# lukedan/libfluid

Measured on AMD Instinct MI355X. Metric: particle_steps_per_sec, higher is better.
Workload: dtype f32

## Files before the change

libfluid_amd/csrc/core.hip:

```cpp
#include <math.h>

#include <algorithm>
#include <stdarg.h>
#include <stdio.h>
#include <string.h>

#include <mutex>

#include "common.h"
#include "pcg.h"
#include "stream_set.h"

static thread_local std::string g_create_error;

int lfa_fail(lfa_sim *s, int code, const char *fmt, ...) {
	char buf[512];
	va_list ap;
	va_start(ap, fmt);
	vsnprintf(buf, sizeof buf, fmt, ap);
	va_end(ap);
	if (s) s->err = buf;
	else g_create_error = buf;
	return code;
}
// ... 744 lines not shown
	return LFA_OK;
}

__global__ void k_set_solid(const int32_t *xyz, size_t k, uint8_t *solid, uint8_t *ctype, GridDims g) {
	size_t i = (size_t)blockIdx.x * blockDim.x + threadIdx.x;
	if (i >= k) return;
	int x = xyz[3 * i], y = xyz[3 * i + 1], z = xyz[3 * i + 2];
	if (!in_grid(g, x, y, z)) return;
	uint32_t b = blocked_index(g, x, y, z);
	solid[b] = 1;
	ctype[b] = CT_SOLID;
}

extern "C" int lfa_set_solid_cells(lfa_sim *s, const int32_t *xyz, uint64_t k) {
	if (!s || (!xyz && k)) return LFA_E_INVALID;
	++s->solid_epoch;
	if (k == 0) return LFA_OK;
	LFA_HIP(s, hipSetDevice(s->device));
	LFA_TRY(lfa_corr_commit(s));
	LFA_TRY(lfa_ensure_io(s, k * 12));
	LFA_HIP(s, hipMemcpyAsync(s->io_buf, xyz, k * 12, hipMemcpyHostToDevice, s->stream));
	hipLaunchKernelGGL(k_set_solid, dim3((unsigned)((k + 255) / 256)), dim3(256), 0, s->stream,
	                   (const int32_t *)s->io_buf, (size_t)k, s->solid, s->ctype, s->g);
	LFA_LAUNCH_CHECK(s);
	LFA_HIP(s, hipStreamSynchronize(s->stream));
	s->system_valid = false;
	return LFA_OK;
}

extern "C" int lfa_clear_solid_cells(lfa_sim *s) {
	if (!s) return LFA_E_INVALID;
	++s->solid_epoch;
	LFA_HIP(s, hipSetDevice(s->device));
	LFA_TRY(lfa_corr_commit(s));
	hipLaunchKernelGGL(k_init_ctype, dim3((unsigned)((s->ncp + 255) / 256)), dim3(256), 0, s->stream, s->ctype, s->solid,
	                   s->g, s->ncp);
	LFA_LAUNCH_CHECK(s);
	s->system_valid = false;
	s->grid_valid = false;
	return LFA_OK;
}

struct CellAos {
	double vel[3];
	uint8_t type;
	uint8_t pad[7];
};

__global__ void k_export_cells(CellAos *out, GridDims g, size_t nc, CellView cv) {
	size_t r = (size_t)blockIdx.x * blockDim.x + threadIdx.x;
	if (r >= nc) return;
	int x = (int)(r % g.nx), y = (int)((r / g.nx) % g.ny), z = (int)(r / ((size_t)g.nx * g.ny));
	uint32_t b = blocked_index(g, x, y, z);
	CellAos c;
	memset(&c, 0, sizeof c);
	const int rule = cell_tile_rule(cv, b >> 9);
#pragma unroll
	for (int k = 0; k < 3; ++k) c.vel[k] = cell_velocity(cv, rule, b, k);
	c.type = cell_type(cv, rule, b);
	out[r] = c;
}

static int export_cells(lfa_sim *s, void *aos32, const float *u, const float *v, const float *w, bool old) {
	LFA_HIP(s, hipSetDevice(s->device));
	LFA_TRY(lfa_ensure_io(s, s->nc * 32));
	hipLaunchKernelGGL(k_export_cells, dim3((unsigned)((s->nc + 255) / 256)), dim3(256), 0, s->stream,
	                   (CellAos *)s->io_buf, s->g, s->nc, lfa_cell_view(s, u, v, w, old));
	LFA_LAUNCH_CHECK(s);
	LFA_HIP(s, hipMemcpyAsync(aos32, s->io_buf, s->nc * 32, hipMemcpyDeviceToHost, s->stream));
	LFA_HIP(s, hipStreamSynchronize(s->stream));
	return LFA_OK;
}

extern "C" int lfa_download_cells(lfa_sim *s, void *aos32) {
	if (!s || !aos32) return LFA_E_INVALID;
	return export_cells(s, aos32, s->u, s->v, s->w, false);
}
extern "C" int lfa_download_old_cells(lfa_sim *s, void *aos32) {
	if (!s || !aos32) return LFA_E_INVALID;
	if (!s->uo) return lfa_fail(s, LFA_E_INVALID, "no old grid: FLIP P2G has not run");
	return export_cells(s, aos32, s->uo, s->vo, s->wo, true);
}

__global__ void k_import_cells(const CellAos *in, GridDims g, size_t nc, float *u, float *v, float *w, uint8_t *ctype,
                               uint8_t *solid) {
	size_t r = (size_t)blockIdx.x * blockDim.x + threadIdx.x;
	if (r >= nc) return;
	int x = (int)(r % g.nx), y = (int)((r / g.nx) % g.ny), z = (int)(r / ((size_t)g.nx * g.ny));
	uint32_t b = blocked_index(g, x, y, z);
	CellAos c = in[r];
	u[b] = (float)c.vel[0]; v[b] = (float)c.vel[1]; w[b] = (float)c.vel[2];
	ctype[b] = c.type & 7;
	solid[b] = (c.type & CT_SOLID) ? 1 : 0;
}

extern "C" int lfa_upload_cells(lfa_sim *s, const void *aos32) {
	if (!s || !aos32) return LFA_E_INVALID;
	++s->solid_epoch;
	LFA_HIP(s, hipSetDevice(s->device));
	LFA_TRY(lfa_corr_join(s));
	LFA_TRY(lfa_ensure_io(s, s->nc * 32));
	LFA_HIP(s, hipMemcpyAsync(s->io_buf, aos32, s->nc * 32, hipMemcpyHostToDevice, s->stream));
	hipLaunchKernelGGL(k_import_cells, dim3((unsigned)((s->nc + 255) / 256)), dim3(256), 0, s->stream,
	                   (const CellAos *)s->io_buf, s->g, s->nc, s->u, s->v, s->w, s->ctype, s->solid);
	LFA_LAUNCH_CHECK(s);
	LFA_HIP(s, hipStreamSynchronize(s->stream));
	s->grid_valid = false;
	s->bg[0] = s->bg[1] = s->bg[2] = 0.0;
	s->system_valid = false;
	return LFA_OK;
}

__global__ void __launch_bounds__(256) k_tile_count(const uint32_t *key, size_t n, uint32_t *tile_count, uint32_t *rank) {
	const int lane = threadIdx.x & 63;
	const size_t wave = ((size_t)blockIdx.x * blockDim.x + threadIdx.x) >> 6;
	const size_t i0 = wave * (64 * TC_CHUNKS) + lane;
	uint32_t tile[TC_CHUNKS], my_rank[TC_CHUNKS];
#pragma unroll
	for (int c = 0; c < TC_CHUNKS; ++c) {
		const size_t i = i0 + 64 * c;
		const uint32_t k = i < n ? key[i] : 0xFFFFFFFFu;
		tile[c] = k != 0xFFFFFFFFu ? k >> 9 : 0xFFFFFFFFu;
	}
	lfa_wave_tile_ranks(tile, tile_count, my_rank);
#pragma unroll
	for (int c = 0; c < TC_CHUNKS; ++c) {
		const size_t i = i0 + 64 * c;
		if (tile[c] != 0xFFFFFFFFu) rank[i] = my_rank[c];
	}
}

__global__ void k_tile_flags(const uint32_t *tile_count, uint32_t *flag, int nt) {
	int t = blockIdx.x * blockDim.x + threadIdx.x;
	if (t < nt) flag[t] = tile_count[t] > 0 ? 1u : 0u;
}
__global__ void k_compact_tiles(const uint32_t *flag, const uint32_t *scan, int *list, int *slot_of, int nt) {
	int t = blockIdx.x * blockDim.x + threadIdx.x;
	if (t >= nt) return;
	if (flag[t]) {
		list[scan[t]] = t;
		if (slot_of) slot_of[t] = (int)scan[t];
	} else if (slot_of) {
		slot_of[t] = -1;
	}
}
__global__ void k_dilate(const int *ptiles, int n_ptiles, uint32_t *flag, GridDims g) {
	int i = blockIdx.x * blockDim.x + threadIdx.x;
	if (i >= n_ptiles * 27) return;
	int t = ptiles[i / 27], o = i % 27, tx, ty, tz;
	tile_coords(g, t, tx, ty, tz);
	int x = tx + o % 3 - 1, y = ty + (o / 3) % 3 - 1, z = tz + o / 9 - 1;
	if ((unsigned)x < (unsigned)g.ntx && (unsigned)y < (unsigned)g.nty && (unsigned)z < (unsigned)g.ntz)
		flag[x + g.ntx * (y + g.nty * z)] = 1u;
}

__global__ void k_tile_scatter(size_t n, ParticleSoA src, ParticleSoA dst, const uint32_t *rank,
                               const uint32_t *tile_start, const uint32_t *tile_count, int shuffle, uint32_t *from) {
	size_t i = (size_t)blockIdx.x * blockDim.x + threadIdx.x;
	if (i >= n) return;
	uint32_t key = src.key[i], tile = key >> 9, r = rank[i];
	if (key == 0xFFFFFFFFu) return;
	if (shuffle) {
		uint32_t cnt = tile_count[tile];
		if (cnt % 1000003u != 0) r = (uint32_t)(((uint64_t)r * 1000003ull) % cnt);
	}
	size_t d = (size_t)tile_start[tile] + r;
	dst.key[d] = key;
#pragma unroll
	for (int k = 0; k < 3; ++k) dst.t[k][d] = src.t[k][i];
	dst.id[d] = src.id[i];
	from[d] = (uint32_t)i;
}
__global__ void k_c_to_home(size_t n, ParticleSoA p, float *home, size_t stride) {
	size_t i = (size_t)blockIdx.x * blockDim.x + threadIdx.x;
	if (i >= n || p.key[i] == 0xFFFFFFFFu) return;
	const size_t j = p.id[i];
#pragma unroll
	for (int k = 0; k < 9; ++k) home[k * stride + j] = p.c[k][i];
}
__global__ void k_c_from_home(size_t n, ParticleSoA p, const float *home, size_t stride) {
	size_t i = (size_t)blockIdx.x * blockDim.x + threadIdx.x;
	if (i >= n || p.key[i] == 0xFFFFFFFFu) return;
	const size_t j = p.id[i];
#pragma unroll
	for (int k = 0; k < 9; ++k) p.c[k][i] = home[k * stride + j];
}
__global__ void k_gather_vc(size_t n, ParticleSoA old, ParticleSoA cur, const uint32_t *from, int with_c) {
	size_t d = (size_t)blockIdx.x * blockDim.x + threadIdx.x;
	if (d >= n) return;
	const uint32_t i = from[d];
#pragma unroll
	for (int k = 0; k < 3; ++k) cur.v[k][d] = old.v[k][i];
	if (with_c) {
#pragma unroll
		for (int k = 0; k < 9; ++k) cur.c[k][d] = old.c[k][i];
	}
}

__global__ void __launch_bounds__(256)
k_cell_count(const int *dtiles, int n_dtiles, const uint32_t *key, const uint32_t *tile_start, uint32_t *cell_count) {
	__shared__ uint32_t cnt[LFA_TILE_CELLS];
	for (int slot = blockIdx.x; slot < n_dtiles; slot += gridDim.x) {
		int tile = dtiles[slot];
		cnt[threadIdx.x] = 0;
		cnt[threadIdx.x + 256] = 0;
		__syncthreads();
		uint32_t b = tile_start[tile], e = tile_start[tile + 1];
		for (uint32_t i = b + threadIdx.x; i < e; i += 256) atomicAdd(&cnt[key[i] & 511], 1u);
		__syncthreads();
		cell_count[(size_t)tile * LFA_TILE_CELLS + threadIdx.x] = cnt[threadIdx.x];
		cell_count[(size_t)tile * LFA_TILE_CELLS + 256 + threadIdx.x] = cnt[threadIdx.x + 256];
		__syncthreads();
	}
}

__global__ void k_compact_range(const uint32_t *flag, const uint32_t *scan, int *list, int *slot_of, int lo, int hi,
                                int slot_base) {
	int t = lo + blockIdx.x * blockDim.x + threadIdx.x;
	if (t >= hi) return;
	if (flag[t]) {
		list[scan[t]] = t;
		if (slot_of) slot_of[t] = slot_base + (int)scan[t];
	} else if (slot_of) {
		slot_of[t] = -1;
	}
}
__global__ void k_fill_i32(int *p, int n, int v) {
	int i = blockIdx.x * blockDim.x + threadIdx.x;
	if (i < n) p[i] = v;
}
__global__ void k_gather_u32(const uint32_t *src, const int *idx, int n, uint32_t *dst) {
	int i = threadIdx.x;
	if (i < n) dst[i] = src[idx[i]];
}

__global__ void k_dilate_slots(const int *tile_pslot, uint32_t *flag, GridDims g) {
	const int t = blockIdx.x * blockDim.x + threadIdx.x;
	if (t >= g.nt || tile_pslot[t] < 0) return;
	int tx, ty, tz;
	tile_coords(g, t, tx, ty, tz);
	for (int o = 0; o < 27; ++o) {
		const int x = tx + o % 3 - 1, y = ty + (o / 3) % 3 - 1, z = tz + o / 9 - 1;
		if ((unsigned)x < (unsigned)g.ntx && (unsigned)y < (unsigned)g.nty && (unsigned)z < (unsigned)g.ntz)
			flag[x + g.ntx * (y + g.nty * z)] = 1u;
	}
}

static int compact_tiles_async(lfa_sim *s, const uint32_t *flag, int lo, int hi, int *list, int *slot_of, uint32_t *total_dev) {
	LFA_TRY(lfa_exclusive_scan_u32(s, flag + lo, s->tile_scan + lo, (size_t)(hi - lo), total_dev));
	hipLaunchKernelGGL(k_compact_range, dim3((hi - lo + 255) / 256), dim3(256), 0, s->stream, flag, s->tile_scan - 0,
	                   list - 0, slot_of, lo, hi, 0);
	LFA_LAUNCH_CHECK(s);
	return LFA_OK;
}

int lfa_c_home_ensure(lfa_sim *s, size_t n) {
	if (n <= s->c_home_cap) return LFA_OK;
	const size_t cap = ((n + n / 8) + 1023) & ~(size_t)1023;
	float *nh = nullptr;
	LFA_HIP(s, hipMalloc(&nh, cap * 9 * sizeof(float)));
	auto fail = [&](hipError_t e, const char *what) {
		(void)hipFree(nh);
		return lfa_fail(s, LFA_E_HIP, "%s failed: %s", what, hipGetErrorString(e));
	};
	if (s->c_home && s->c_home_valid && s->c_home_cap)
		for (int k = 0; k < 9; ++k) {
			const hipError_t e = hipMemcpyAsync(nh + (size_t)k * cap, s->c_home + (size_t)k * s->c_home_cap,
			                                    s->c_home_cap * 4, hipMemcpyDeviceToDevice, s->stream);
			if (e != hipSuccess) return fail(e, "copying C to its larger home array");
		}
	if (s->c_home) {
		const hipError_t e = hipStreamSynchronize(s->stream);
		if (e != hipSuccess) return fail(e, "hipStreamSynchronize");
		LFA_HIP(s, hipFree(s->c_home));
	}
	s->c_home = nh;
	s->c_home_cap = cap;
	return LFA_OK;
}
int lfa_c_home_restore(lfa_sim *s) {
	if (!s->c_home_valid) return LFA_OK;
	s->c_home_valid = false;
	const size_t n = s->binned ? s->np_live : s->np;
	if (!n) return LFA_OK;
	hipLaunchKernelGGL(k_c_from_home, dim3((unsigned)((n + 255) / 256)), dim3(256), 0, s->stream, n, s->pb[s->cur], (const float *)s->c_home,
	                   s->c_home_cap);
	LFA_LAUNCH_CHECK(s);
	return LFA_OK;
}

int lfa_particles_materialize(lfa_sim *s) {
	if (!s->vc_pending) return LFA_OK;
	LFA_TRY(lfa_corr_commit(s));
	s->vc_pending = false;
	LFA_HIP(s, hipSetDevice(s->device));
	const size_t n = s->np_live;
	if (!n) return LFA_OK;
	hipLaunchKernelGGL(k_gather_vc, dim3((unsigned)((n + 255) / 256)), dim3(256), 0, s->stream, n, s->pb[s->cur ^ 1], s->pb[s->cur],
	                   (const uint32_t *)s->vc_src, s->vc_with_c ? 1 : 0);
	LFA_LAUNCH_CHECK(s);
	return LFA_OK;
}

extern "C" int lfa_hash_particles(lfa_sim *s) { return lfa_hash_particles_impl(s, false); }
int lfa_hash_particles_impl(lfa_sim *s, bool counts_done) {
	if (!s) return LFA_E_INVALID;
	LFA_HIP(s, hipSetDevice(s->device));
	LFA_TRY(lfa_corr_commit(s));
	LFA_TRY(lfa_particles_materialize(s));
	const GridDims &g = s->g;
	const int nt = g.nt, L = g.ntx * g.nty;
	const size_t n = s->binned ? s->np_live : s->np;
	ParticleSoA &src = s->pb[s->cur], &dst = s->pb[s->cur ^ 1];
	const int own_lo = s->slab_lo * L, own_hi = s->slab_hi * L;
	const int all_lo = lfa_has_lo(s) ? own_lo - L : own_lo, all_hi = lfa_has_hi(s) ? own_hi + L : own_hi;

	if (!counts_done) {
		LFA_HIP(s, hipMemsetAsync(s->tile_count, 0, (size_t)(nt + 1) * 4, s->stream));
		if (n) {
			hipLaunchKernelGGL(k_tile_count, dim3((unsigned)((n + 256 * TC_CHUNKS - 1) / (256 * TC_CHUNKS))), dim3(256), 0, s->stream, src.key, n,
			                   s->tile_count, s->rank);
			LFA_LAUNCH_CHECK(s);
		}
	}
	LFA_TRY(lfa_exclusive_scan_u32(s, s->tile_count, s->tile_start, (size_t)nt + 1, nullptr));
	LFA_HIP(s, hipMemcpyAsync(s->h_pinned + 8, s->tile_start + nt, 4, hipMemcpyDeviceToHost, s->stream));

	hipLaunchKernelGGL(k_tile_flags, dim3((nt + 255) / 256), dim3(256), 0, s->stream, s->tile_count, s->tile_flag, nt);
	LFA_LAUNCH_CHECK(s);
	LFA_TRY(lfa_dist_exchange_tile_layers_u32(s, s->tile_flag));
	hipLaunchKernelGGL(k_fill_i32, dim3((nt + 255) / 256), dim3(256), 0, s->stream, s->tile_pslot, nt, -1);
	LFA_LAUNCH_CHECK(s);
	const bool one_sync = !s->dist;
	if (one_sync) {
		uint32_t *tot = (uint32_t *)s->pcg_state + 8;
		LFA_TRY(compact_tiles_async(s, s->tile_flag, 0, nt, s->ptiles_all, s->tile_pslot, tot));
		LFA_HIP(s, hipMemsetAsync(s->tile_flag, 0, (size_t)(nt + 1) * 4, s->stream));
		hipLaunchKernelGGL(k_dilate_slots, dim3((nt + 255) / 256), dim3(256), 0, s->stream, (const int *)s->tile_pslot, s->tile_flag, g);
		LFA_LAUNCH_CHECK(s);
		LFA_TRY(compact_tiles_async(s, s->tile_flag, 0, nt, s->dtiles, nullptr, tot + 1));
		LFA_HIP(s, hipMemcpyAsync(s->h_pinned + 9, tot, 8, hipMemcpyDeviceToHost, s->stream));
		LFA_HIP(s, hipStreamSynchronize(s->stream));
		s->n_ptiles_all = (int)s->h_pinned[9];
		s->n_dtiles = (int)s->h_pinned[10];
		s->p_off = 0;
		s->n_ptiles = s->n_ptiles_all;
		s->n_own_first = s->n_own_last = s->n_ghost_lo = s->n_ghost_hi = 0;
		s->ptiles = s->ptiles_all;
	} else {
		uint32_t *tot = (uint32_t *)s->pcg_state + 20;
		LFA_TRY(compact_tiles_async(s, s->tile_flag, all_lo, all_hi, s->ptiles_all, s->tile_pslot, tot));
		int marks[4] = {own_lo, own_lo + L < own_hi ? own_lo + L : own_hi, own_hi - L > own_lo ? own_hi - L : own_lo, own_hi};
		int *didx = s->pcg_state + 12;
		LFA_HIP(s, hipMemcpyAsync(didx, marks, 16, hipMemcpyHostToDevice, s->stream));
		hipLaunchKernelGGL(k_gather_u32, dim3(1), dim3(64), 0, s->stream, s->tile_scan, didx, 4, tot + 1);
		LFA_LAUNCH_CHECK(s);
		LFA_HIP(s, hipMemsetAsync(s->tile_flag, 0, (size_t)(nt + 1) * 4, s->stream));
		hipLaunchKernelGGL(k_dilate_slots, dim3((nt + 255) / 256), dim3(256), 0, s->stream, (const int *)s->tile_pslot, s->tile_flag, g);
		LFA_LAUNCH_CHECK(s);
		if (own_lo > 0) LFA_HIP(s, hipMemsetAsync(s->tile_flag, 0, (size_t)own_lo * 4, s->stream));
		if (own_hi < nt) LFA_HIP(s, hipMemsetAsync(s->tile_flag + own_hi, 0, (size_t)(nt - own_hi) * 4, s->stream));
		LFA_TRY(lfa_dist_exchange_tile_layers_u32(s, s->tile_flag));
		LFA_TRY(compact_tiles_async(s, s->tile_flag, own_lo, own_hi, s->dtiles, nullptr, tot + 5));
		{
			const int hlo[4] = {s->slab_lo * L, (s->slab_hi - 1) * L, (s->slab_lo - 1) * L, s->slab_hi * L};
			const bool on[4] = {lfa_has_lo(s), lfa_has_hi(s), lfa_has_lo(s), lfa_has_hi(s)};
			LFA_HIP(s, hipMemsetAsync(tot + 6, 0, 16, s->stream));
			for (int w = 0; w < 4; ++w)
				if (on[w]) LFA_TRY(compact_tiles_async(s, s->tile_flag, hlo[w], hlo[w] + L, s->halo_tiles + (size_t)w * L, nullptr, tot + 6 + w));
		}
		LFA_HIP(s, hipMemcpyAsync(s->h_pinned + 20, tot, 40, hipMemcpyDeviceToHost, s->stream));
		LFA_HIP(s, hipStreamSynchronize(s->stream));
		const uint32_t *h = s->h_pinned + 20;
		s->n_ptiles_all = (int)h[0];
		int vals[4];
		for (int k = 0; k < 4; ++k) vals[k] = marks[k] >= all_hi ? s->n_ptiles_all : (int)h[1 + k];
		s->p_off = vals[0];
		s->n_ptiles = vals[3] - vals[0];
		s->n_own_first = vals[1] - vals[0];
		s->n_own_last = vals[3] - vals[2];
		s->n_ghost_lo = s->p_off;
		s->n_ghost_hi = s->n_ptiles_all - vals[3];
		s->ptiles = s->ptiles_all + s->p_off;
		s->n_dtiles = (int)h[5];
		for (int w = 0; w < 4; ++w) s->n_halo[w] = (int)h[6 + w];
	}
	s->np_live = s->h_pinned[8];
	if (s->dist) s->np = s->np_live;
	s->holes = false;
	s->n_arrivals = 0;
	s->move_pending = false;
	if (n) {
		const dim3 sgrid((unsigned)((n + 255) / 256));
		const bool home = s->prm.simulation_method != LFA_APIC;
		if (home && !s->c_home_valid) {
			LFA_TRY(lfa_c_home_ensure(s, s->dist ? std::max<size_t>(s->pcap, (size_t)s->next_global_id) : s->pcap));
			hipLaunchKernelGGL(k_c_to_home, sgrid, dim3(256), 0, s->stream, n, src, s->c_home, s->c_home_cap);
			LFA_LAUNCH_CHECK(s);
			s->c_home_valid = true;
		} else if (!home && s->c_home_valid) {
			LFA_TRY(lfa_c_home_restore(s));
		}
		hipLaunchKernelGGL(k_tile_scatter, sgrid, dim3(256), 0, s->stream, n, src, dst, s->rank, s->tile_start, s->tile_count,
		                   s->binned ? 0 : 1, s->vc_src);
		LFA_LAUNCH_CHECK(s);
		s->cur ^= 1;
		s->vc_pending = true;
		s->vc_extent = n;
		s->vc_with_c = !home;
	}
	if (s->n_dtiles) {
		int grid = s->n_dtiles < 8192 ? s->n_dtiles : 8192;
		hipLaunchKernelGGL(k_cell_count, dim3(grid), dim3(256), 0, s->stream, s->dtiles, s->n_dtiles,
		                   s->pb[s->cur].key, s->tile_start, s->cell_count);
		LFA_LAUNCH_CHECK(s);
	}
	s->binned = true;
	s->system_valid = false;
	s->unknown_count_valid = false;
	return LFA_OK;
}

int lfa_dist_build_halo_lists(lfa_sim *s, const uint32_t *flag, int *lists, int n[4]) {
	const int L = s->g.ntx * s->g.nty;
	const int lo[4] = {s->slab_lo * L, (s->slab_hi - 1) * L, (s->slab_lo - 1) * L, s->slab_hi * L};
	const bool on[4] = {lfa_has_lo(s), lfa_has_hi(s), lfa_has_lo(s), lfa_has_hi(s)};
	uint32_t *tot = (uint32_t *)s->pcg_state + 26;
	LFA_HIP(s, hipMemsetAsync(tot, 0, 16, s->stream));
	for (int w = 0; w < 4; ++w)
		if (on[w]) LFA_TRY(compact_tiles_async(s, flag, lo[w], lo[w] + L, lists + (size_t)w * L, nullptr, tot + w));
	LFA_HIP(s, hipMemcpyAsync(s->h_pinned + 26, tot, 16, hipMemcpyDeviceToHost, s->stream));
	LFA_HIP(s, hipStreamSynchronize(s->stream));
	for (int w = 0; w < 4; ++w) n[w] = (int)s->h_pinned[26 + w];
	return LFA_OK;
}

__global__ void k_raw_unknown_flags(GridDims g, size_t nc, const uint32_t *cell_count, const uint32_t *tile_flag,
                                    uint32_t *flag, int z0, int z1) {
	size_t r = (size_t)blockIdx.x * blockDim.x + threadIdx.x;
	if (r >= nc) return;
	int x = (int)(r % g.nx), y = (int)((r / g.nx) % g.ny), z = (int)(r / ((size_t)g.nx * g.ny));
	uint32_t b = blocked_index(g, x, y, z);
	flag[r] = (z >= z0 && z < z1 && tile_flag[b >> 9] && cell_count[b] > 0) ? 1u : 0u;
}

int lfa_number_unknowns(lfa_sim *s) {
	if (s->unknown_count_valid) return LFA_OK;
	if (!s->binned) return lfa_fail(s, LFA_E_INVALID, "call lfa_hash_particles first");
	if (!s->raw_scan) LFA_HIP(s, hipMalloc(&s->raw_scan, (s->nc + 1) * 4));
	hipLaunchKernelGGL(k_raw_unknown_flags, dim3((unsigned)((s->nc + 255) / 256)), dim3(256), 0, s->stream, s->g, s->nc,
	                   s->cell_count, s->tile_flag, s->raw_scan, s->slab_lo * 8, s->slab_hi * 8);
	LFA_LAUNCH_CHECK(s);
	LFA_TRY(lfa_exclusive_scan_u32(s, s->raw_scan, s->raw_scan, s->nc, (uint32_t *)s->pcg_state + 10));
	LFA_HIP(s, hipMemcpyAsync(s->h_pinned, (uint32_t *)s->pcg_state + 10, 4, hipMemcpyDeviceToHost, s->stream));
	LFA_HIP(s, hipStreamSynchronize(s->stream));
	s->n_unknowns = s->h_pinned[0];
	s->unknown_count_valid = true;
	return LFA_OK;
}

extern "C" uint64_t lfa_num_fluid_cells(lfa_sim *s) {
	if (!s || lfa_number_unknowns(s) != LFA_OK) return 0;
	return s->n_unknowns;
}

__global__ void k_export_fluid_cells(GridDims g, size_t nc, const uint32_t *cell_count, const uint32_t *tile_flag,
                                     const uint32_t *raw_scan, uint64_t *out, int z0, int z1) {
	size_t r = (size_t)blockIdx.x * blockDim.x + threadIdx.x;
	if (r >= nc) return;
	int x = (int)(r % g.nx), y = (int)((r / g.nx) % g.ny), z = (int)(r / ((size_t)g.nx * g.ny));
	uint32_t b = blocked_index(g, x, y, z);
	if (z >= z0 && z < z1 && tile_flag[b >> 9] && cell_count[b] > 0) out[raw_scan[r]] = r;
}

extern "C" int lfa_download_fluid_cells(lfa_sim *s, uint64_t *raw, uint64_t n) {
	if (!s || (!raw && n)) return LFA_E_INVALID;
	LFA_HIP(s, hipSetDevice(s->device));
	LFA_TRY(lfa_number_unknowns(s));
	if (n != s->n_unknowns) return lfa_fail(s, LFA_E_INVALID, "fluid cell count is %llu", (unsigned long long)s->n_unknowns);
	if (n == 0) return LFA_OK;
	LFA_TRY(lfa_ensure_io(s, n * 8));
	hipLaunchKernelGGL(k_export_fluid_cells, dim3((unsigned)((s->nc + 255) / 256)), dim3(256), 0, s->stream, s->g, s->nc,
	                   s->cell_count, s->tile_flag, s->raw_scan, (uint64_t *)s->io_buf, s->slab_lo * 8, s->slab_hi * 8);
	LFA_LAUNCH_CHECK(s);
	LFA_HIP(s, hipMemcpyAsync(raw, s->io_buf, n * 8, hipMemcpyDeviceToHost, s->stream));
	LFA_HIP(s, hipStreamSynchronize(s->stream));
	return LFA_OK;
}

__global__ void k_export_counts(GridDims g, size_t nc, const uint32_t *cell_count, const uint32_t *tile_flag,
                                uint32_t *out) {
	size_t r = (size_t)blockIdx.x * blockDim.x + threadIdx.x;
	if (r >= nc) return;
	int x = (int)(r % g.nx), y = (int)((r / g.nx) % g.ny), z = (int)(r / ((size_t)g.nx * g.ny));
	uint32_t b = blocked_index(g, x, y, z);
	out[r] = tile_flag[b >> 9] ? cell_count[b] : 0u;
}

extern "C" int lfa_download_cell_counts(lfa_sim *s, uint32_t *count) {
	if (!s || !count) return LFA_E_INVALID;
	if (!s->binned) return lfa_fail(s, LFA_E_INVALID, "call lfa_hash_particles first");
	LFA_HIP(s, hipSetDevice(s->device));
	LFA_TRY(lfa_ensure_io(s, s->nc * 4));
	hipLaunchKernelGGL(k_export_counts, dim3((unsigned)((s->nc + 255) / 256)), dim3(256), 0, s->stream, s->g, s->nc,
	                   s->cell_count, s->tile_flag, (uint32_t *)s->io_buf);
	LFA_LAUNCH_CHECK(s);
	LFA_HIP(s, hipMemcpyAsync(count, s->io_buf, s->nc * 4, hipMemcpyDeviceToHost, s->stream));
	LFA_HIP(s, hipStreamSynchronize(s->stream));
	return LFA_OK;
}

__global__ void __launch_bounds__(256) k_max_speed2(size_t n, const float *vx, const float *vy, const float *vz, double *partials) {
	__shared__ double lds[4];
	double m = 0.0;
	for (size_t i = (size_t)blockIdx.x * 256 + threadIdx.x; i < n; i += (size_t)gridDim.x * 256) {
		double x = vx[i], y = vy[i], z = vz[i];
		double l = x * x + y * y + z * z;
		m = l > m ? l : m;
	}
	m = wave_max(m);
	if ((threadIdx.x & 63) == 0) lds[threadIdx.x >> 6] = m;
	__syncthreads();
	if (threadIdx.x == 0) {
		for (int i = 1; i < 4; ++i) m = lds[i] > m ? lds[i] : m;
		partials[blockIdx.x] = m;
	}
}

extern "C" int lfa_cfl(lfa_sim *s, double *out) {
	if (!s || !out) return LFA_E_INVALID;
	LFA_HIP(s, hipSetDevice(s->device));
	LFA_TRY(lfa_corr_join(s));
	double m = 0.0;
	if (s->vmax2_valid && s->np_live) {
		LFA_HIP(s, hipStreamSynchronize(s->stream));
		float f;
		memcpy(&f, s->h_pinned + 100, 4);
		m = (double)f;
	} else if (s->np_live) {
		LFA_TRY(lfa_particles_materialize(s));
		int grid = (int)((s->np_live + 255) / 256);
		if (grid > 1024) grid = 1024;
		const ParticleSoA &p = s->pb[s->cur];
		hipLaunchKernelGGL(k_max_speed2, dim3(grid), dim3(256), 0, s->stream, s->np_live, p.v[0], p.v[1], p.v[2], s->partials);
		LFA_LAUNCH_CHECK(s);
		std::vector<double> h(grid);
		LFA_HIP(s, hipMemcpyAsync(h.data(), s->partials, grid * 8, hipMemcpyDeviceToHost, s->stream));
		LFA_HIP(s, hipStreamSynchronize(s->stream));
		for (double x : h) m = x > m ? x : m;
	}
	*out = s->prm.cell_size / sqrt(m);
	return LFA_OK;
}

template <int U, bool NT>
__global__ void __launch_bounds__(256) k_stream_copy(const float4 *in, float4 *out, size_t n) {
	const size_t chunk = (size_t)256 * U;
	for (size_t base = (size_t)blockIdx.x * chunk; base < n; base += (size_t)gridDim.x * chunk) {
		float4 v[U];
#pragma unroll
		for (int k = 0; k < U; ++k) {
			const size_t i = base + (size_t)k * 256 + threadIdx.x;
			if (i < n) {
				if (NT) {
					typedef float f4v __attribute__((ext_vector_type(4)));
					const f4v w = __builtin_nontemporal_load((const f4v *)in + i);
					v[k] = make_float4(w.x, w.y, w.z, w.w);
				} else {
					v[k] = in[i];
				}
			}
		}
#pragma unroll
		for (int k = 0; k < U; ++k) {
			const size_t i = base + (size_t)k * 256 + threadIdx.x;
			if (i < n) {
				if (NT) {
					typedef float f4v __attribute__((ext_vector_type(4)));
					f4v w;
					w.x = v[k].x; w.y = v[k].y; w.z = v[k].z; w.w = v[k].w;
					__builtin_nontemporal_store(w, (f4v *)out + i);
				} else {
					out[i] = v[k];
				}
			}
		}
	}
}
template <int U>
__global__ void __launch_bounds__(256) k_stream_read(const float4 *in, float *sink, size_t n) {
	float acc = 0.f;
	const size_t chunk = (size_t)256 * U;
	for (size_t base = (size_t)blockIdx.x * chunk; base < n; base += (size_t)gridDim.x * chunk) {
		float4 v[U];
#pragma unroll
		for (int k = 0; k < U; ++k) {
			const size_t i = base + (size_t)k * 256 + threadIdx.x;
			v[k] = i < n ? in[i] : make_float4(0.f, 0.f, 0.f, 0.f);
		}
#pragma unroll
		for (int k = 0; k < U; ++k) acc += (v[k].x + v[k].y) + (v[k].z + v[k].w);
	}
	if (acc == 123.456f) sink[0] = acc;
}

static int g_stream_best = -1;
extern "C" const char *lfa_bench_stream_variant(void) {
	static const char *names[] = {"1 x float4 per thread and iteration", "4 x float4 in flight", "4 x float4 in flight, non-temporal",
	                              "8 x float4 in flight, non-temporal", "4 x float4 in flight, non-temporal, 32 workgroups per CU"};
	return g_stream_best >= 0 ? names[g_stream_best] : "";
}

extern "C" int lfa_bench_stream(lfa_sim *s, uint64_t bytes, int reps, double *copy_gbs, double *read_gbs) {
	if (!s || reps < 1 || bytes < (1u << 20)) return LFA_E_INVALID;
	LFA_HIP(s, hipSetDevice(s->device));
	const size_t n = (size_t)bytes / 16;
	float4 *a = nullptr, *b = nullptr;
	hipEvent_t e0 = nullptr, e1 = nullptr;
	auto cleanup = [&]() {
		if (e0) (void)hipEventDestroy(e0);
		if (e1) (void)hipEventDestroy(e1);
		if (a) (void)(hipFree)(a);
		if (b) (void)(hipFree)(b);
	};
	if ((hipMalloc)((void **)&a, n * 16) != hipSuccess || (hipMalloc)((void **)&b, n * 16) != hipSuccess) {
		cleanup();
		return lfa_fail(s, LFA_E_OOM, "lfa_bench_stream: hipMalloc of 2 x %llu bytes failed", (unsigned long long)bytes);
	}
	int rc = LFA_OK;
	auto run = [&]() -> int {
		LFA_HIP(s, hipEventCreate(&e0));
		LFA_HIP(s, hipEventCreate(&e1));
		LFA_HIP(s, hipMemsetAsync(a, 0, n * 16, s->stream));
		LFA_HIP(s, hipMemsetAsync(b, 0, n * 16, s->stream));
		float ms = 0.f;
		double best_copy = 0.0, best_read = 0.0;
		for (int variant = 0; variant < 7; ++variant) {
			const dim3 grid(256 * (variant == 4 ? 32 : 16));
			for (int r = -1; r < reps; ++r) {
				if (r == 0) LFA_HIP(s, hipEventRecord(e0, s->stream));
				switch (variant) {
				case 0: hipLaunchKernelGGL((k_stream_copy<1, false>), grid, dim3(256), 0, s->stream, (const float4 *)a, b, n); break;
				case 1: hipLaunchKernelGGL((k_stream_copy<4, false>), grid, dim3(256), 0, s->stream, (const float4 *)a, b, n); break;
				case 2: hipLaunchKernelGGL((k_stream_copy<4, true>), grid, dim3(256), 0, s->stream, (const float4 *)a, b, n); break;
				case 3: hipLaunchKernelGGL((k_stream_copy<8, true>), grid, dim3(256), 0, s->stream, (const float4 *)a, b, n); break;
				case 4: hipLaunchKernelGGL((k_stream_copy<4, true>), grid, dim3(256), 0, s->stream, (const float4 *)a, b, n); break;
				case 5: hipLaunchKernelGGL(k_stream_read<1>, grid, dim3(256), 0, s->stream, (const float4 *)a, (float *)b, n); break;
				default: hipLaunchKernelGGL(k_stream_read<4>, grid, dim3(256), 0, s->stream, (const float4 *)a, (float *)b, n); break;
				}
			}
			LFA_LAUNCH_CHECK(s);
			LFA_HIP(s, hipEventRecord(e1, s->stream));
			LFA_HIP(s, hipEventSynchronize(e1));
			LFA_HIP(s, hipEventElapsedTime(&ms, e0, e1));
			const double gbs = (double)(n * 16) * reps * (variant < 5 ? 2.0 : 1.0) / ((double)ms * 1e-3) * 1e-9;
			if (variant < 5 && gbs > best_copy) { best_copy = gbs; g_stream_best = variant; }
			if (variant >= 5 && gbs > best_read) best_read = gbs;
		}
		if (copy_gbs) *copy_gbs = best_copy;
		if (read_gbs) *read_gbs = best_read;
		return LFA_OK;
	};
	rc = run();
	cleanup();
	return rc;
}

extern "C" int lfa_enable_timing(lfa_sim *s, int on) {
	if (!s) return LFA_E_INVALID;
	LFA_HIP(s, hipSetDevice(s->device));
	if (on && !s->ev_created) {
		for (auto &e : s->ev) LFA_HIP(s, hipEventCreate(&e));
		s->ev_created = true;
	}
	s->timing = on != 0;
	return LFA_OK;
}
extern "C" int lfa_get_timings(lfa_sim *s, double ms[LFA_NUM_TIMERS]) {
	if (!s || !ms) return LFA_E_INVALID;
	for (int i = 0; i < LFA_NUM_TIMERS; ++i) ms[i] = s->ms[i];
	return LFA_OK;
}
extern "C" int lfa_get_counts(lfa_sim *s, uint64_t counts[5]) {
	if (!s || !counts) return LFA_E_INVALID;
	counts[0] = s->np;
	counts[1] = lfa_num_fluid_cells(s);
	counts[2] = (uint64_t)s->n_ptiles;
	counts[3] = (uint64_t)s->n_dtiles;
	counts[4] = s->ncp;
	return LFA_OK;
}
```

Baseline: 5.222 billion.

## Overlap tile-list compaction with particle scatter on a second stream

In the single-device path, tile flag, compaction and dilation work is forked onto a secondary stream via events, while the particle scatter (and c_home conversion) is enqueued on the main stream at the same time. The host then waits only on the join event before reading the tile counts, instead of synchronizing the whole main stream before the scatter is launched. This aims to hide the latency of the small compaction kernels and the host round-trip behind the scatter, at the cost of extra event handling and swapping the stream pointer temporarily.

```diff
diff --git a/libfluid_amd/csrc/core.hip b/libfluid_amd/csrc/core.hip
--- a/libfluid_amd/csrc/core.hip
+++ b/libfluid_amd/csrc/core.hip
@@ -1070,6 +1070,48 @@
 	return LFA_OK;
 }
 
+static int build_tile_lists(lfa_sim *s) {
+	const GridDims &g = s->g;
+	const int nt = g.nt;
+	const dim3 tgrid((nt + 255) / 256);
+	uint32_t *tot = (uint32_t *)s->pcg_state + 8;
+	LFA_HIP(s, hipMemcpyAsync(s->h_pinned + 8, s->tile_start + nt, 4, hipMemcpyDeviceToHost, s->stream));
+	hipLaunchKernelGGL(k_tile_flags, tgrid, dim3(256), 0, s->stream, s->tile_count, s->tile_flag, nt);
+	LFA_LAUNCH_CHECK(s);
+	hipLaunchKernelGGL(k_fill_i32, tgrid, dim3(256), 0, s->stream, s->tile_pslot, nt, -1);
+	LFA_LAUNCH_CHECK(s);
+	LFA_TRY(compact_tiles_async(s, s->tile_flag, 0, nt, s->ptiles_all, s->tile_pslot, tot));
+	LFA_HIP(s, hipMemsetAsync(s->tile_flag, 0, (size_t)(nt + 1) * 4, s->stream));
+	hipLaunchKernelGGL(k_dilate_slots, tgrid, dim3(256), 0, s->stream, (const int *)s->tile_pslot, s->tile_flag, g);
+	LFA_LAUNCH_CHECK(s);
+	LFA_TRY(compact_tiles_async(s, s->tile_flag, 0, nt, s->dtiles, nullptr, tot + 1));
+	LFA_HIP(s, hipMemcpyAsync(s->h_pinned + 9, tot, 8, hipMemcpyDeviceToHost, s->stream));
+	return LFA_OK;
+}
+
+static int scatter_to_tiles(lfa_sim *s, size_t n) {
+	if (!n) return LFA_OK;
+	ParticleSoA &src = s->pb[s->cur], &dst = s->pb[s->cur ^ 1];
+	const dim3 sgrid((unsigned)((n + 255) / 256));
+	const bool home = s->prm.simulation_method != LFA_APIC;
+	if (home && !s->c_home_valid) {
+		LFA_TRY(lfa_c_home_ensure(s, s->dist ? std::max<size_t>(s->pcap, (size_t)s->next_global_id) : s->pcap));
+		hipLaunchKernelGGL(k_c_to_home, sgrid, dim3(256), 0, s->stream, n, src, s->c_home, s->c_home_cap);
+		LFA_LAUNCH_CHECK(s);
+		s->c_home_valid = true;
+	} else if (!home && s->c_home_valid) {
+		LFA_TRY(lfa_c_home_restore(s));
+	}
+	hipLaunchKernelGGL(k_tile_scatter, sgrid, dim3(256), 0, s->stream, n, src, dst, s->rank, s->tile_start, s->tile_count,
+	                   s->binned ? 0 : 1, s->vc_src);
+	LFA_LAUNCH_CHECK(s);
+	s->cur ^= 1;
+	s->vc_pending = true;
+	s->vc_extent = n;
+	s->vc_with_c = !home;
+	return LFA_OK;
+}
+
 extern "C" int lfa_hash_particles(lfa_sim *s) { return lfa_hash_particles_impl(s, false); }
 int lfa_hash_particles_impl(lfa_sim *s, bool counts_done) {
 	if (!s) return LFA_E_INVALID;
@@ -1079,7 +1121,7 @@
 	const GridDims &g = s->g;
 	const int nt = g.nt, L = g.ntx * g.nty;
 	const size_t n = s->binned ? s->np_live : s->np;
-	ParticleSoA &src = s->pb[s->cur], &dst = s->pb[s->cur ^ 1];
+	ParticleSoA &src = s->pb[s->cur];
 	const int own_lo = s->slab_lo * L, own_hi = s->slab_hi * L;
 	const int all_lo = lfa_has_lo(s) ? own_lo - L : own_lo, all_hi = lfa_has_hi(s) ? own_hi + L : own_hi;
 
@@ -1092,23 +1134,24 @@
 		}
 	}
 	LFA_TRY(lfa_exclusive_scan_u32(s, s->tile_count, s->tile_start, (size_t)nt + 1, nullptr));
-	LFA_HIP(s, hipMemcpyAsync(s->h_pinned + 8, s->tile_start + nt, 4, hipMemcpyDeviceToHost, s->stream));
-
-	hipLaunchKernelGGL(k_tile_flags, dim3((nt + 255) / 256), dim3(256), 0, s->stream, s->tile_count, s->tile_flag, nt);
-	LFA_LAUNCH_CHECK(s);
-	LFA_TRY(lfa_dist_exchange_tile_layers_u32(s, s->tile_flag));
-	hipLaunchKernelGGL(k_fill_i32, dim3((nt + 255) / 256), dim3(256), 0, s->stream, s->tile_pslot, nt, -1);
-	LFA_LAUNCH_CHECK(s);
+
 	const bool one_sync = !s->dist;
 	if (one_sync) {
-		uint32_t *tot = (uint32_t *)s->pcg_state + 8;
-		LFA_TRY(compact_tiles_async(s, s->tile_flag, 0, nt, s->ptiles_all, s->tile_pslot, tot));
-		LFA_HIP(s, hipMemsetAsync(s->tile_flag, 0, (size_t)(nt + 1) * 4, s->stream));
-		hipLaunchKernelGGL(k_dilate_slots, dim3((nt + 255) / 256), dim3(256), 0, s->stream, (const int *)s->tile_pslot, s->tile_flag, g);
-		LFA_LAUNCH_CHECK(s);
-		LFA_TRY(compact_tiles_async(s, s->tile_flag, 0, nt, s->dtiles, nullptr, tot + 1));
-		LFA_HIP(s, hipMemcpyAsync(s->h_pinned + 9, tot, 8, hipMemcpyDeviceToHost, s->stream));
-		LFA_HIP(s, hipStreamSynchronize(s->stream));
+		LFA_HIP(s, hipEventRecord(s->ev_fork, s->stream));
+		LFA_HIP(s, hipStreamWaitEvent(s->stream2, s->ev_fork, 0));
+		hipStream_t main_stream = s->stream;
+		s->stream = s->stream2;
+		int rc = build_tile_lists(s);
+		s->stream = main_stream;
+		const hipError_t e_join = hipEventRecord(s->ev_join, s->stream2);
+		if (rc == LFA_OK && e_join == hipSuccess) rc = scatter_to_tiles(s, n);
+		hipError_t e_wait = hipSuccess;
+		if (rc == LFA_OK && e_join == hipSuccess) e_wait = hipEventSynchronize(s->ev_join);
+		const hipError_t e_order = e_join == hipSuccess ? hipStreamWaitEvent(s->stream, s->ev_join, 0) : hipStreamSynchronize(s->stream2);
+		if (rc < 0) return rc;
+		LFA_HIP(s, e_join);
+		LFA_HIP(s, e_wait);
+		LFA_HIP(s, e_order);
 		s->n_ptiles_all = (int)s->h_pinned[9];
 		s->n_dtiles = (int)s->h_pinned[10];
 		s->p_off = 0;
@@ -1116,6 +1159,12 @@
 		s->n_own_first = s->n_own_last = s->n_ghost_lo = s->n_ghost_hi = 0;
 		s->ptiles = s->ptiles_all;
 	} else {
+		LFA_HIP(s, hipMemcpyAsync(s->h_pinned + 8, s->tile_start + nt, 4, hipMemcpyDeviceToHost, s->stream));
+		hipLaunchKernelGGL(k_tile_flags, dim3((nt + 255) / 256), dim3(256), 0, s->stream, s->tile_count, s->tile_flag, nt);
+		LFA_LAUNCH_CHECK(s);
+		LFA_TRY(lfa_dist_exchange_tile_layers_u32(s, s->tile_flag));
+		hipLaunchKernelGGL(k_fill_i32, dim3((nt + 255) / 256), dim3(256), 0, s->stream, s->tile_pslot, nt, -1);
+		LFA_LAUNCH_CHECK(s);
 		uint32_t *tot = (uint32_t *)s->pcg_state + 20;
 		LFA_TRY(compact_tiles_async(s, s->tile_flag, all_lo, all_hi, s->ptiles_all, s->tile_pslot, tot));
 		int marks[4] = {own_lo, own_lo + L < own_hi ? own_lo + L : own_hi, own_hi - L > own_lo ? own_hi - L : own_lo, own_hi};
@@ -1158,25 +1207,7 @@
 	s->holes = false;
 	s->n_arrivals = 0;
 	s->move_pending = false;
-	if (n) {
-		const dim3 sgrid((unsigned)((n + 255) / 256));
-		const bool home = s->prm.simulation_method != LFA_APIC;
-		if (home && !s->c_home_valid) {
-			LFA_TRY(lfa_c_home_ensure(s, s->dist ? std::max<size_t>(s->pcap, (size_t)s->next_global_id) : s->pcap));
-			hipLaunchKernelGGL(k_c_to_home, sgrid, dim3(256), 0, s->stream, n, src, s->c_home, s->c_home_cap);
-			LFA_LAUNCH_CHECK(s);
-			s->c_home_valid = true;
-		} else if (!home && s->c_home_valid) {
-			LFA_TRY(lfa_c_home_restore(s));
-		}
-		hipLaunchKernelGGL(k_tile_scatter, sgrid, dim3(256), 0, s->stream, n, src, dst, s->rank, s->tile_start, s->tile_count,
-		                   s->binned ? 0 : 1, s->vc_src);
-		LFA_LAUNCH_CHECK(s);
-		s->cur ^= 1;
-		s->vc_pending = true;
-		s->vc_extent = n;
-		s->vc_with_c = !home;
-	}
+	if (!one_sync) LFA_TRY(scatter_to_tiles(s, n));
 	if (s->n_dtiles) {
 		int grid = s->n_dtiles < 8192 ? s->n_dtiles : 8192;
 		hipLaunchKernelGGL(k_cell_count, dim3(grid), dim3(256), 0, s->stream, s->dtiles, s->n_dtiles,
```

Result: no change. 5.240 billion (median of 2 runs) (+0.3%).
